# olydis/vlg_matching

Measured on AMD Instinct MI355X. Metric: vlg_queries_per_sec, higher is better.
Workload: dtype u32

## Files before the change

### vlg_matching_amd/csrc/join_device.hpp

```cpp
#pragma once
namespace {

constexpr uint32_t kNone = 0xFFFFFFFFu;
constexpr uint32_t kChecksumSlots = 64;

struct SegMeta {
    uint32_t begin, end;
    uint32_t pbegin, pend;
    uint32_t dist;
    uint32_t level;
    uint32_t next;
    uint32_t query;
    uint64_t lo, hi;
};

struct QueryMeta {
    uint32_t seg0;
    uint32_t k;
    uint64_t end_len;
    uint64_t out_first;
    uint64_t out_tuple;
};

__device__ __forceinline__ uint64_t sat_add(uint64_t a, uint64_t b) { uint64_t c = a + b; return c < a ? ~0ull : c; }
// ... 381 lines not shown
        }
        out[i] = v;
    }
}

template <typename pos_t>
__global__ void __launch_bounds__(256) join_init_kernel(const pos_t* __restrict__ P, const uint32_t* __restrict__ seg_begin, uint32_t nseg,
                                                        const SegMeta* __restrict__ sm, uint64_t r0, uint64_t r1, uint64_t* __restrict__ fbits,
                                                        pos_t* __restrict__ endp)
{
    const uint32_t lane = threadIdx.x & 63;
    const uint64_t wave = ((uint64_t)blockIdx.x * blockDim.x + threadIdx.x) >> 6;
    const uint64_t run_begin = r0 + wave * kRun;
    if (run_begin >= r1) return;
    const uint64_t run_end = run_begin + kRun < r1 ? run_begin + kRun : r1;
    uint32_t s_w = seg_find(seg_begin, nseg, run_begin);
    for (uint64_t base = run_begin; base < run_end; base += 64) {
        const uint64_t e = base + lane;
        if (e < run_end) {
            uint32_t s = s_w;
            while (seg_begin[s + 1] <= e) ++s;
            const SegMeta m = sm[s];
            endp[e] = P[phys_of(m, (uint32_t)e)];
            s_w = s;
        }
        const unsigned long long act = __ballot(e < run_end);
        if (lane == 0) fbits[base >> 6] = act;
        s_w = __shfl(s_w, 0);
    }
}

template <typename pos_t, bool kLast>
__device__ __forceinline__ bool link_finish(const pos_t* __restrict__ P, const SegMeta& nx, const FeasRef& fb, uint32_t e, bool want, uint32_t j,
                                            pos_t v, pos_t thi, pos_t* __restrict__ endp, uint32_t* __restrict__ link)
{
    bool ok = false;
    if (want && j < nx.pend) {
        if (kLast) {
            ok = v <= thi;
            if (ok) { if (link) link[e] = j; endp[e] = v; }
        } else {
            const uint32_t at = nx.begin + (j - nx.pbegin);
            const uint32_t ej = next_feasible(fb, at);
            if (ej < nx.end) {
                const pos_t pv = ej == at ? v : P[phys_of(nx, ej)];
                if (pv <= thi) { ok = true; if (link) link[e] = ej; endp[e] = endp[ej]; }
            }
        }
    }
    return ok;
}

template <typename pos_t, bool kLast>
__global__ void __launch_bounds__(256) join_link_kernel(const pos_t* __restrict__ P, const pos_t* __restrict__ F ,
                                                        const uint32_t* __restrict__ seg_begin, uint32_t nseg,
                                                        const SegMeta* __restrict__ sm, uint32_t r0, uint32_t r1,
                                                        FeasRef fb, uint64_t* __restrict__ fbits_out,
                                                        pos_t* __restrict__ endp, uint32_t* __restrict__ link)
{
    const uint32_t lane = threadIdx.x & 63;
    const uint64_t wave = ((uint64_t)blockIdx.x * blockDim.x + threadIdx.x) >> 6;
    if (wave * kLinkRun >= (uint64_t)(r1 - r0)) return;
    const uint32_t run_begin = r0 + (uint32_t)wave * kLinkRun;
    const uint32_t run_end = r1 - run_begin > kLinkRun ? run_begin + kLinkRun : r1;
    uint32_t s_w = wave_seg_find(seg_begin, nseg, run_begin);
    uint32_t seg_end = seg_begin[s_w + 1];
    SegMeta m = sm[s_w], nx = sm[m.next];
    uint32_t hint_seg = kNone, hint = 0;
    pos_t x_pre = 0, x_pre1 = 0;
    bool have_pre = false, have_pre1 = false;
    for (uint32_t base = run_begin; base < run_end; base += 64) {
        if (base >= seg_end) {
            while (seg_begin[s_w + 1] <= base) ++s_w;
            seg_end = seg_begin[s_w + 1];
            m = sm[s_w]; nx = sm[m.next];
            have_pre = false; have_pre1 = false;
        }
        if (run_end - base >= 128 && base + 127 < seg_end) {
            const uint32_t e0 = base + lane, e1 = e0 + 64;
            const pos_t x0 = have_pre ? x_pre : P[phys_of(m, e0)];
            const pos_t x1 = have_pre1 ? x_pre1 : P[phys_of(m, e1)];
            const uint32_t left = run_end - base - 128;
            const uint32_t room = seg_end - base - 128;
            have_pre = left > 0 && (left < 64 ? left : 64u) <= room;
            have_pre1 = left >= 128 && room >= 128;
            if (have_pre) x_pre = e0 + 128 < run_end ? P[phys_of(m, e0 + 128)] : (pos_t)0;
            if (have_pre1) x_pre1 = P[phys_of(m, e1 + 128)];
            pos_t tlo0, thi0, tlo1, thi1, v0 = 0, v1 = 0;
            const bool want0 = gap_window<pos_t>((uint64_t)x0, nx.lo, nx.hi, tlo0, thi0);
            const bool want1 = gap_window<pos_t>((uint64_t)x1, nx.lo, nx.hi, tlo1, thi1);
            uint32_t j0 = nx.pend, j1 = nx.pend;
            if (hint_seg != s_w)
                hint = wave_kary_lower_bound(P, F, nx.pbegin, nx.pend, (uint64_t)__shfl(tlo0, 0));
            wave_lower_bound2(P, F, hint, nx.pend, tlo0, want0, tlo1, want1, j0, v0, j1, v1);
            if (!want0) j0 = nx.pend;
            if (!want1) j1 = nx.pend;
            const bool ok0 = link_finish<pos_t, kLast>(P, nx, fb, e0, want0, j0, v0, thi0, endp, link);
            const bool ok1 = link_finish<pos_t, kLast>(P, nx, fb, e1, want1, j1, v1, thi1, endp, link);
            const unsigned long long okm0 = __ballot(ok0), okm1 = __ballot(ok1);
            if (lane == 0) { fbits_out[base >> 6] = okm0; fbits_out[(base >> 6) + 1] = okm1; }
            hint_seg = s_w;
            hint = __shfl(j1, 63);
            base += 64;
            continue;
        }
        have_pre1 = false;
        const uint32_t e = base + lane;
        const bool active = e < run_end;
        const uint32_t step_last = run_end - base > 64 ? base + 63 : run_end - 1;
        uint32_t j = 0, s_last = s_w;
        if (step_last < seg_end) {
            const pos_t x = have_pre ? x_pre : (active ? P[phys_of(m, e)] : (pos_t)0);
            const uint32_t en = e + 64;
            have_pre = run_end - base > 64 && (run_end - base > 128 ? base + 127 : run_end - 1) < seg_end;
            if (have_pre) x_pre = en < run_end ? P[phys_of(m, en)] : (pos_t)0;
            pos_t tlo, thi, v = 0;
            const bool want = gap_window<pos_t>((uint64_t)x, nx.lo, nx.hi, tlo, thi) && active;
            j = nx.pend;
            if (hint_seg != s_w) hint = wave_kary_lower_bound(P, F, nx.pbegin, nx.pend, (uint64_t)__shfl(tlo, 0));
            j = wave_lower_bound(P, F, hint, nx.pend, tlo, want, v);
            if (!want) j = nx.pend;
            const bool ok = link_finish<pos_t, kLast>(P, nx, fb, e, want, j, v, thi, endp, link);
            const unsigned long long okm = __ballot(ok);
            if (lane == 0) fbits_out[base >> 6] = okm;
        } else {
            have_pre = false;
            uint32_t s = s_w;
            bool ok = false;
            if (active) {
                while (seg_begin[s + 1] <= e) ++s;
                const SegMeta ml = sm[s];
                const SegMeta nl = sm[ml.next];
                const uint64_t x = P[phys_of(ml, e)];
                const uint64_t tlo = sat_add(x, nl.lo), thi = sat_add(x, nl.hi);
                j = gallop_lower_bound(P, (s == hint_seg) ? hint : nl.pbegin, nl.pend, tlo);
                if (e < ml.end) {
                    if (kLast) {
                        ok = j < nl.pend && (uint64_t)P[j] <= thi;
                        if (ok) { if (link) link[e] = j; endp[e] = P[j]; }
                    } else if (j < nl.pend) {
                        const uint32_t ej = next_feasible(fb, (uint64_t)nl.begin + (j - nl.pbegin));
                        if (ej < nl.end && (uint64_t)P[phys_of(nl, ej)] <= thi) { ok = true; if (link) link[e] = ej; endp[e] = endp[ej]; }
                    }
                }
            }
            const unsigned long long okm = __ballot(ok);
            if (lane == 0) fbits_out[base >> 6] = okm;
            s_last = __shfl(s, (int)(step_last - base));
        }
        hint_seg = s_last;
        hint = __shfl(j, (int)(step_last - base));
    }
}

template <typename pos_t>
__global__ void __launch_bounds__(256) join_jump_kernel(const pos_t* __restrict__ P, const pos_t* __restrict__ F, const uint32_t* __restrict__ seg_begin, uint32_t nseg,
                                                        const SegMeta* __restrict__ sm, const QueryMeta* __restrict__ qm, uint64_t r0,
                                                        uint64_t r1, FeasRef fb, const pos_t* __restrict__ endp,
                                                        uint32_t* __restrict__ jump, uint32_t* __restrict__ qstart)
{
    __shared__ pos_t s_tile[4][kTB];
    const uint32_t lane = threadIdx.x & 63, wv = threadIdx.x >> 6;
    const uint64_t wave = uniform(((uint64_t)blockIdx.x * blockDim.x + threadIdx.x) >> 6);
    const uint64_t run_begin = r0 + wave * kRun;
    if (run_begin >= r1) return;
    const uint64_t run_end = run_begin + kRun < r1 ? run_begin + kRun : r1;
    pos_t* tile = s_tile[wv];
    uint32_t s = wave_seg_find(seg_begin, nseg, run_begin);
    uint64_t cur = run_begin;
    while (cur < run_end) {
        while (seg_begin[s + 1] <= cur) ++s;
        const SegMeta m = sm[s];
        const uint64_t seg_end = seg_begin[s + 1];
        if (m.level != 0) {
            const uint64_t piece_end = run_end < seg_end ? run_end : seg_end;
            for (uint64_t a = cur + lane; a < piece_end; a += 64) jump[a] = kNone;
            cur = piece_end;
        } else if (m.end - m.begin >= kMinPiece && cur < m.end) {
            const uint64_t piece_end = run_end < m.end ? run_end : (uint64_t)m.end;
            const uint64_t end_len = qm[m.query].end_len;
            if (cur == m.begin && lane == 0) { const uint32_t me = next_feasible(fb, cur); qstart[m.query] = me < m.end ? me : kNone; }
            uint32_t fence = 0;
            for (uint64_t blk0 = cur; blk0 < piece_end; blk0 += kBlk) {
                const uint64_t blk1 = blk0 + kBlk < piece_end ? blk0 + kBlk : piece_end;
                pos_t key[kKeys], v[kKeys];
                uint32_t j[kKeys];
                uint32_t need = 0;
#pragma unroll
                for (uint32_t i = 0; i < kKeys; ++i) {
                    const uint64_t a = blk0 + lane + 64 * i;
                    key[i] = 0;
                    if (a < blk1 && is_feasible(fb, a)) {
                        pos_t unused;
                        if (gap_window<pos_t>((uint64_t)endp[a], end_len, end_len, key[i], unused)) need |= 1u << i;
                    }
                }
                const uint32_t own = phys_of(m, (uint32_t)blk0) + 1;
                fence = fence > own ? fence : own;
                const uint32_t asked = need;
                tile_lower_bounds<pos_t>(P, F, fence, m.pend, tile, key, need, j, v);
                uint32_t jm = fence;
#pragma unroll
                for (uint32_t i = 0; i < kKeys; ++i) {
                    const uint64_t a = blk0 + lane + 64 * i;
                    if (a < blk1) {
                        uint32_t out = kNone;
                        if ((asked >> i) & 1) {
                            jm = j[i] > jm ? j[i] : jm;
                            if (j[i] < m.pend) {
                                const uint32_t ej = next_feasible(fb, (uint64_t)m.begin + (j[i] - m.pbegin));
                                if (ej < m.end) out = ej;
                            }
                        }
                        jump[a] = out;
                    }
                }
                jm = wave_max_u32(jm);
                fence = jm;
            }
            cur = piece_end;
        } else {
            const uint64_t e = cur + lane;
            const uint64_t grp_end = cur + 64 < run_end ? cur + 64 : run_end;
            if (e < grp_end) {
                uint32_t sl = s;
                while (seg_begin[sl + 1] <= e) ++sl;
                const SegMeta ml = sm[sl];
                uint32_t out = kNone;
                if (ml.level == 0 && e < ml.end) {
                    if (is_feasible(fb, e)) {
                        const uint64_t lim = sat_add((uint64_t)endp[e], qm[ml.query].end_len);
                        const uint32_t jp = gallop_lower_bound(P, phys_of(ml, (uint32_t)e) + 1, ml.pend, lim);
                        if (jp < ml.pend) {
                            const uint32_t ej = next_feasible(fb, (uint64_t)ml.begin + (jp - ml.pbegin));
                            if (ej < ml.end) out = ej;
                        }
                    }
                    if ((uint32_t)e == ml.begin) { const uint32_t me = next_feasible(fb, e); qstart[ml.query] = me < ml.end ? me : kNone; }
                }
                jump[e] = out;
            }
            cur = grp_end;
        }
    }
}

constexpr uint32_t kTile = 1024;

__global__ void __launch_bounds__(256) chain_tiles_kernel(const uint32_t* __restrict__ jump, uint64_t t0 ,
                                                          uint64_t r1, uint2* __restrict__ xh)
{
    static_assert(kTile == 1024, "the packed word holds 10-bit tile offsets");
    __shared__ uint32_t s_ext[kTile];
    __shared__ uint32_t s_st[2][kTile];
    constexpr uint32_t kDone = 1u << 10;
    const uint64_t base = t0 + (uint64_t)blockIdx.x * kTile;
    const uint64_t tile_end = base + kTile;
    uint32_t st[4];
    bool open = false;
#pragma unroll
    for (uint32_t r = 0; r < 4; ++r) {
        const uint32_t li = threadIdx.x + 256 * r;
        const uint64_t e = base + li;
        const uint32_t j = e < r1 ? jump[e] : kNone;
        const bool inside = j != kNone && (uint64_t)j < tile_end;
        s_ext[li] = j;
        st[r] = (inside ? (uint32_t)(j - base) : kDone) | (li << 21);
        s_st[0][li] = st[r];
        open |= inside;
    }
    uint32_t cur = 0;
    for (uint32_t round = 0; round < 10 && __syncthreads_or(open); ++round) {
        open = false;
#pragma unroll
        for (uint32_t r = 0; r < 4; ++r) {
            const uint32_t li = threadIdx.x + 256 * r;
            if (!(st[r] & kDone)) {
                const uint32_t nx = s_st[cur][st[r] & 1023u];
                const uint32_t hops = ((st[r] >> 11) & 1023u) + ((nx >> 11) & 1023u) + 1;
                st[r] = (nx & 0x7FFu) | (hops << 11) | (nx & (1023u << 21));
                open |= !(st[r] & kDone);
            }
            s_st[cur ^ 1][li] = st[r];
        }
        cur ^= 1;
    }
    __syncthreads();
#pragma unroll
    for (uint32_t r = 0; r < 4; ++r) {
        const uint32_t li = threadIdx.x + 256 * r;
        const uint64_t e = base + li;
        if (e < r1) xh[e] = make_uint2(s_ext[st[r] >> 21], ((st[r] >> 11) & 1023u) + 1);
    }
}

__global__ void chain_walk_kernel(const SegMeta* __restrict__ sm, const QueryMeta* __restrict__ qm, uint32_t nq,
                                  const uint32_t* __restrict__ qstart, const uint2* __restrict__ xh, const uint32_t* __restrict__ rec_begin,
                                  uint2* __restrict__ records, uint32_t* __restrict__ rec_count, unsigned long long* __restrict__ counts)
{
    uint32_t q = blockIdx.x * blockDim.x + threadIdx.x;
    if (q >= nq) return;
    const QueryMeta Q = qm[q];
    unsigned long long n_match = 0;
    uint32_t nrec = 0;
    if (Q.seg0 != kNone) {
        const uint32_t mbegin = sm[Q.seg0].begin;
        uint2* rec = records + rec_begin[q];
        uint32_t cur = qstart[q];
        while (cur != kNone) {
            uint2 v = xh[cur];
            rec[nrec++] = make_uint2(cur, mbegin + (uint32_t)n_match);
            n_match += v.y;
            cur = v.x;
        }
    }
    rec_count[q] = nrec;
    counts[q] = n_match;
}

__global__ void __launch_bounds__(256) chain_emit_kernel(const uint32_t* __restrict__ rec_begin, const uint32_t* __restrict__ rec_count,
                                                         const uint2* __restrict__ records, uint32_t total_rec_slots,
                                                         const uint32_t* __restrict__ rec_query, const uint32_t* __restrict__ jump,
                                                         const uint2* __restrict__ xh, uint64_t r1 ,
                                                         uint32_t* __restrict__ mlist)
{
    constexpr uint16_t kOut = 0xFFFFu;
    constexpr uint32_t kPer = kTile / 64;
    __shared__ uint16_t s_t[4][2][kTile];
    const uint32_t lane = threadIdx.x & 63, wv = threadIdx.x >> 6;
    const uint32_t r = uniform((uint32_t)(((uint64_t)blockIdx.x * blockDim.x + threadIdx.x) >> 6));
    if (r >= total_rec_slots) return;
    const uint32_t q = rec_query[r];
    if (r - rec_begin[q] >= rec_count[q]) return;
    const uint2 rc = records[r];
    const uint64_t tile_base = (uint64_t)(rc.x / kTile) * kTile;
    const uint32_t cnt = uniform(xh[rc.x].y);
#pragma unroll
    for (uint32_t i = 0; i < kPer; ++i) {
        const uint64_t e = tile_base + lane + 64 * i;
        const uint32_t j = e < r1 ? jump[e] : kNone;
        s_t[wv][0][lane + 64 * i] = (j != kNone && (uint64_t)j < tile_base + kTile) ? (uint16_t)(j - (uint32_t)tile_base) : kOut;
// ... 94 lines not shown
```

### vlg_matching_amd/csrc/search.hip

```cpp
#include <algorithm>
#include <chrono>
#include <cstdio>
#include <cstdlib>
#include <cstring>
#include <mutex>
#include <numeric>
#include <thread>
#include <unordered_map>
#include <string.h>
#include <string>
#include <vector>
#include "common.hpp"
#include "kernels.hpp"
#include <rocprim/rocprim.hpp>

using namespace vlg;

#include "search_types.hpp"
#include "filter_shape.hpp"
#include "window_cut.hpp"
#include "shape_dispatch.hpp"

enum { KS_BSEARCH = 0, KS_EXPAND, KS_LOCATE, KS_LOCATE_PART, KS_LOCATE_RESOLVE, KS_SORT, KS_FILTER_LADDER, KS_FILTER_PIVOT, KS_FILTER_PASS, KS_FILTER_COMPACT,
       KS_JOIN_INIT, KS_JOIN_LINK, KS_JOIN_SCAN, KS_JOIN_CHAIN, KS_GATHER, KS_EXCHANGE, KS_WINDOW_CUT, KS_CLASS_SEARCH, KS_COUNT };
static const char* kKernelNames[KS_COUNT] = {"backward_search", "expand", "locate", "locate_partition", "locate_resolve", "sort", "filter_ladder", "filter_pivot",
                                             "filter_pass", "filter_compact", "join_init", "join_link", "join_scan", "join_chain", "gather", "exchange", "window_cut", "class_search"};

struct vlg_workspace {
    hipStream_t stream = nullptr;
    uint64_t cap_bytes = 0;
    uint8_t* arena = nullptr;
    uint64_t arena_bytes = 0;
    HostPool host;
    bool profile = false;
    bool dedup = true;
    bool sweep = true;
    bool tuples = true;
    bool trail = true;
    bool filter = true;
    uint64_t filter_min = 1ull << 12;
    uint64_t filter_stream_min = 1ull << 16;
    bool filter_pivot = true;
    uint64_t filter_group_bytes = 0;
    uint64_t filter_pivot_ratio = 3;
    uint64_t pivot_range_ratio = 16;
    uint32_t compact_dense_min = 256;
    uint32_t pivot_rungs = 1;
    int list_sort = 1;
    uint64_t global_sort_min = 1ull << 20;
    bool quad_walk = true;
    uint64_t sweep_min = 1ull << 22;
    uint64_t sweep_tail = 1ull << 22;
    uint32_t unsample_pct = 0;
    uint64_t unsample_min = 1ull << 28;
    uint64_t unsample_tail = 1ull << 20;
    uint32_t class_intervals = 1024;
    uint64_t sample_reads = 0;
    uint8_t* head = nullptr;
    uint64_t head_bytes = 0;
    uint64_t tmp_key[6] = {0, 0, 0, 0, 0, 0};
    size_t tmp_bytes = 0;
    int x_ranks = 1, x_rank = 0;
    vlg_exchange_fn x_fn = nullptr;
    vlg_alltoall_fn x_a2a = nullptr;
    void* x_ctx = nullptr;
    void* x_comm = nullptr;
    bool exchange_all = false;
    uint64_t* x_status = nullptr;
    uint32_t x_agreed = 0;
    vlg_kernel_stat stats[KS_COUNT];
    std::vector<std::pair<hipEvent_t, hipEvent_t>> pending[KS_COUNT];
    std::vector<hipEvent_t> free_events;
};

namespace {

struct PhaseTrace {
    bool on, sync;
    hipStream_t st;
    std::chrono::steady_clock::time_point t0;
    explicit PhaseTrace(hipStream_t s) : on(getenv("VLG_TRACE") != nullptr), sync(!on || strcmp(getenv("VLG_TRACE"), "host") != 0), st(s), t0(std::chrono::steady_clock::now()) {}
    void mark(const char* what)
    {
// ... 110 lines not shown
}

extern "C" void vlg_workspace_destroy(vlg_workspace* ws)
{
    if (!ws) return;
    ws_collect(ws);
    for (hipEvent_t e : ws->free_events) (void)hipEventDestroy(e);
    if (ws->arena) (void)hipFree(ws->arena);
    if (ws->head) (void)hipFree(ws->head);
    if (ws->x_status) (void)hipFree(ws->x_status);
    ws->host.release();
    delete ws;
}

extern "C" vlg_status vlg_workspace_profile(vlg_workspace* ws, int enable)
{
    if (!ws) return fail(VLG_E_INVALID, "null argument");
    ws_reset_stats(ws);
    ws->profile = enable != 0;
    return VLG_OK;
}

extern "C" vlg_status vlg_workspace_set_option(vlg_workspace* ws, const char* name, int64_t value)
{
    if (!ws || !name) return fail(VLG_E_INVALID, "null argument");
    if (!strcmp(name, "dedup")) { ws->dedup = value != 0; return VLG_OK; }
    if (!strcmp(name, "sweep")) { ws->sweep = value != 0; return VLG_OK; }
    if (!strcmp(name, "sweep_min")) { ws->sweep_min = (uint64_t)value; return VLG_OK; }
    if (!strcmp(name, "global_sort_min")) { ws->global_sort_min = (uint64_t)value; return VLG_OK; }
    if (!strcmp(name, "list_sort")) { ws->list_sort = value > 2 ? 1 : (int)value; return VLG_OK; }
    if (!strcmp(name, "trail")) { ws->trail = value != 0; return VLG_OK; }
    if (!strcmp(name, "quad_walk")) { ws->quad_walk = value != 0; return VLG_OK; }
    if (!strcmp(name, "tuples")) { ws->tuples = value != 0; return VLG_OK; }
    if (!strcmp(name, "filter")) { ws->filter = value != 0; return VLG_OK; }
    if (!strcmp(name, "filter_min")) { ws->filter_min = (uint64_t)value; return VLG_OK; }
    if (!strcmp(name, "filter_pivot")) { ws->filter_pivot = value != 0; return VLG_OK; }
    if (!strcmp(name, "filter_pivot_ratio")) { ws->filter_pivot_ratio = (uint64_t)value; return VLG_OK; }
    if (!strcmp(name, "pivot_range_ratio")) { ws->pivot_range_ratio = (uint64_t)std::max<int64_t>(0, value); return VLG_OK; }
    if (!strcmp(name, "compact_dense_min")) { ws->compact_dense_min = (uint32_t)std::max<int64_t>(0, std::min<int64_t>(value, 1 << 20)); return VLG_OK; }
    if (!strcmp(name, "pivot_rungs")) { ws->pivot_rungs = value <= 0 ? 0u : (value == 1 ? 1u : 2u); return VLG_OK; }
    if (!strcmp(name, "filter_stream_min")) { ws->filter_stream_min = (uint64_t)value; return VLG_OK; }
    if (!strcmp(name, "filter_group_bytes")) { ws->filter_group_bytes = (uint64_t)value; return VLG_OK; }
    if (!strcmp(name, "reserve")) {
        const uint64_t b = std::min<uint64_t>((uint64_t)value, ws->cap_bytes);
        return ws_reserve(ws, b + b / 96 + (256ull << 20));
    }
    if (!strcmp(name, "sweep_tail")) { ws->sweep_tail = (uint64_t)value; return VLG_OK; }
    if (!strcmp(name, "exchange_all")) { ws->exchange_all = value != 0; return VLG_OK; }
    if (!strcmp(name, "unsample_pct")) { ws->unsample_pct = (uint32_t)std::max<int64_t>(0, std::min<int64_t>(value, 1 << 20)); return VLG_OK; }
    if (!strcmp(name, "unsample_tail")) { ws->unsample_tail = (uint64_t)value; return VLG_OK; }
    if (!strcmp(name, "class_intervals")) {
        if (value < 1 || value > (int64_t)kClassIntervalsMax) return fail(VLG_E_INVALID, "class_intervals: 1 .. 2^20");
        ws->class_intervals = (uint32_t)value;
        return VLG_OK;
    }
    if (!strcmp(name, "unsample_min")) { ws->unsample_min = (uint64_t)value; return VLG_OK; }
    return fail(VLG_E_INVALID, std::string("unknown workspace option ") + name);
}

namespace {
vlg_status ws_exchange_reset(vlg_workspace* ws, int n_ranks)
{
    ws->x_comm = nullptr; ws->x_fn = nullptr; ws->x_a2a = nullptr; ws->x_ctx = nullptr; ws->x_ranks = 1; ws->x_rank = 0;
    if (n_ranks > 1 && !ws->x_status) VLG_HIP_TRY(hipMalloc((void**)&ws->x_status, 8 * 1024));
    return VLG_OK;
}
// ... 871 lines not shown
            hipLaunchKernelGGL(HIP_KERNEL_NAME(fence_build_kernel<pos_t>), launch_grid(gacc / 64, 8192), dim3(256), 0, st, L.P, (uint64_t)0, gacc / 64, L.F);
            VLG_HIP_TRY(hipGetLastError());
        }
        return VLG_OK;
    }
};

template <typename pos_t>
vlg_status build_physical(const vlg_index* idx, vlg_workspace* ws, vlg_result* res, const Plan& pl, const SuperChunk& sc, const ChunkPlan& cp, bool wide,
                          Arena& A, unsigned long long* d_stats, Lists<pos_t>& L, const vlg_queries* q = nullptr, const std::vector<uint64_t>* xq = nullptr,
                          Agreement* ag = nullptr)
{
    L.P = L.Pc = L.F = L.R = nullptr; L.pc_cap = 0; L.roff = nullptr;
    PhysicalPass<pos_t> pp{idx, ws, res, pl, cp, wide, A, d_stats, L};
    pp.layout(sc.dlist);
    if (!pp.gacc) return ag ? ag->settle(VLG_OK) : VLG_OK;
    const std::function<vlg_status()> plan_sort = [&pp]() { return pp.plan_sort(); };
    if (vlg_status s = pp.carve()) return s;
    if (vlg_status s = pp.locate(plan_sort)) return s;
    if (vlg_status s = pp.sort(L.P)) return s;
    if (vlg_status s = pp.exchange(L.P, q, xq, ag)) return s;
    if (vlg_status s = pp.check_sort()) return s;
    if (vlg_status s = pp.fences_and_ladder()) return s;
    res->sum.located_occurrences += pp.acc;
    return VLG_OK;
}

}

#include "filter.hpp"

namespace {

template <typename pos_t>
struct JoinChunk {
    const vlg_queries* q; vlg_workspace* ws; vlg_result* res; const uint64_t q0, q1; const Plan& pl; const Lists<pos_t>& L;
    Arena A;
    unsigned long long* d_stats; const FilterGroup* fg;
    hipStream_t st = ws->stream;
    PhaseTrace jt{st};
    const pos_t* P = L.P;
    pos_t* Pc = L.Pc;
    const pos_t* F = L.F;
    const uint64_t s0 = q->qsub[q0], s1 = q->qsub[q1];
    const uint32_t nseg = (uint32_t)(s1 - s0), nq = (uint32_t)(q1 - q0);
    ResultPiece piece{q0, q1};
    bool empty = false;
    svec<QueryMeta> qm;
    uint32_t kmax = 0, nlive = 0, n_rec = 0;
    svec<uint32_t> t_seg, t_cidx; svec<uint64_t> t_run0;
    bool t_kind[2] = {false, false};
    uint64_t pc_total = 0;
    std::vector<uint32_t> cls_count, cls_first;
    std::vector<uint64_t> cls_slot_begin, cls_slot_end;
    svec<SegMeta> sm; svec<uint32_t> seg_begin;
    uint64_t T = 0, lvl0_begin = 0, lvl0_end = 0, t0 = 0;
    svec<uint32_t> rec_begin, rec_query;
    svec<unsigned long long> counts, first_of;
    uint32_t* link = nullptr; pos_t* endp = nullptr;
    FeasBits fb; uint64_t* lvl_ptr[kBitLevels]; FeasBits* d_fb = nullptr; FeasRef fref{nullptr, nullptr};
    uint32_t* jump = nullptr; uint32_t* mlist = nullptr; uint2* xh = nullptr;
    SegMeta* d_sm = nullptr; QueryMeta* d_qm = nullptr; uint32_t* d_segb = nullptr; unsigned long long* d_counts = nullptr;
    uint32_t* d_qstart = nullptr; uint32_t* d_recb = nullptr; uint32_t* d_recc = nullptr; uint32_t* d_recq = nullptr; uint2* d_rec = nullptr;

    uint64_t eo(uint64_t s) const { return fg ? fg->eff[s - fg->sub0] : pl.occ[s]; }
    bool filtered(uint64_t s) const { return fg && fg->cidx[s - fg->sub0] != kNone; }
    bool live(uint64_t qi) const { return q->qsub[qi + 1] > q->qsub[qi] && eo(q->qsub[qi]) > 0; }

    void survivor_tasks()
    {
        qm.resize(nq);
        if (fg) { t_seg.reserve(nseg); t_cidx.reserve(nseg); t_run0.reserve(nseg + 1); }
        t_run0.push_back(0);
        for (uint64_t qi = q0; qi < q1; ++qi) {
            const uint64_t a = q->qsub[qi];
            const uint32_t k = (uint32_t)(q->qsub[qi + 1] - a);
            QueryMeta& Q = qm[qi - q0];
            Q.k = k; Q.end_len = q->end_len[qi]; Q.out_first = Q.out_tuple = 0; Q.seg0 = kNone;
            if (!live(qi)) continue;
            kmax = std::max(kmax, k);
            if (fg && !fg->speculated)
                for (uint32_t i = 0; i < k; ++i) {
                    const uint32_t c = fg->cidx[a + i - fg->sub0];
                    if (c == kNone) continue;
                    t_cidx.push_back(c);
                    t_seg.push_back(fg->cseg[c]);
                    t_kind[fg->ckind[c]] = true;
                    t_run0.push_back(t_run0.back() + (fg->crun0[c + 1] - fg->crun0[c]));
                    pc_total += fg->eff[a + i - fg->sub0];
                }
        }
    }

    vlg_status compact_survivors()
    {
        if (t_seg.empty()) return VLG_OK;
// ... 81 lines not shown
                cnt = (m0.end - 1) / kTile - m0.begin / kTile + 1;
            }
            rec_begin[i + 1] = rec_begin[i] + cnt;
            rec_query.insert(rec_query.end(), cnt, i);
        }
        n_rec = rec_begin[nq];
        empty = lvl0_end <= lvl0_begin;
        t0 = lvl0_begin / kTile * kTile;
    }

    vlg_status carve()
    {
        link = ws->tuples ? A.take<uint32_t>(T) : nullptr;
        endp = A.take<pos_t>(T);
        uint64_t words = (T + 63) / 64 + 1;
        for (uint32_t l = 0; l < kBitLevels; ++l) {
            fb.lvl[l] = lvl_ptr[l] = A.take<uint64_t>(words);
            fb.words[l] = words;
            words = (words + 63) / 64 + 1;
        }
        d_fb = A.take<FeasBits>(1);
        fref = FeasRef{lvl_ptr[0], d_fb};
        const uint64_t n0 = lvl0_end - t0;
        uint32_t* jump_a = A.take<uint32_t>(n0);
        uint32_t* mlist_a = A.take<uint32_t>(n0);
        uint2* xh_a = A.take<uint2>(n0);
        jump = jump_a ? jump_a - t0 : nullptr;
        mlist = mlist_a ? mlist_a - t0 : nullptr;
        xh = xh_a ? xh_a - t0 : nullptr;
        d_sm = A.take<SegMeta>(nlive + 1);
        d_qm = A.take<QueryMeta>(nq);
        d_segb = A.take<uint32_t>(nlive + 2);
        d_counts = A.take<unsigned long long>(nq);
        d_qstart = A.take<uint32_t>(nq);
        d_recb = A.take<uint32_t>(nq + 1);
        d_recc = A.take<uint32_t>(nq);
        d_recq = A.take<uint32_t>(n_rec + 1);
        d_rec = A.take<uint2>(n_rec + 1);
        if (A.failed) return fail(VLG_E_INTERNAL, "arena carve failed (join)");
        return VLG_OK;
    }

    vlg_status upload()
    {
        for (uint32_t l = 0; l < kBitLevels; ++l) VLG_HIP_TRY(hipMemsetAsync(lvl_ptr[l], 0, fb.words[l] * 8, st));
        VLG_HIP_TRY(hipMemcpyAsync(d_fb, &fb, sizeof fb, hipMemcpyHostToDevice, st));
        VLG_HIP_TRY(hipMemcpyAsync(d_recb, rec_begin.data(), (nq + 1) * 4, hipMemcpyHostToDevice, st));
        if (n_rec) VLG_HIP_TRY(hipMemcpyAsync(d_recq, rec_query.data(), n_rec * 4, hipMemcpyHostToDevice, st));
        VLG_HIP_TRY(hipMemsetAsync(d_qstart, 0xFF, nq * 4, st));
        VLG_HIP_TRY(hipMemcpyAsync(d_sm, sm.data(), (nlive + 1) * sizeof(SegMeta), hipMemcpyHostToDevice, st));
        VLG_HIP_TRY(hipMemcpyAsync(d_segb, seg_begin.data(), (nlive + 2) * 4, hipMemcpyHostToDevice, st));
        VLG_HIP_TRY(hipMemcpyAsync(d_qm, qm.data(), nq * sizeof(QueryMeta), hipMemcpyHostToDevice, st));
        return VLG_OK;
    }

    vlg_status summarize_class(uint32_t d)
    {
        const uint64_t b0 = cls_slot_begin[d], b1 = cls_slot_end[d];
        if (b1 <= b0) return VLG_OK;
        Timed t(ws, KS_JOIN_SCAN, (b1 - b0) / 8);
        uint64_t w0 = b0 >> 6, w1 = (b1 + 63) >> 6;
        for (uint32_t l = 1; l < kBitLevels; ++l) {
            w0 >>= 6; w1 = (w1 + 63) >> 6;
            hipLaunchKernelGGL(bits_summary_kernel, launch_grid(w1 - w0, 4096), dim3(256), 0, st, fb.lvl[l - 1], fb.words[l - 1], w0, w1, lvl_ptr[l]);
        }
        VLG_HIP_TRY(hipGetLastError());
        return VLG_OK;
    }

    vlg_status link_classes()
    {
        if (cls_slot_end[0] > cls_slot_begin[0]) {
            Timed t(ws, KS_JOIN_INIT, 0);
            hipLaunchKernelGGL(HIP_KERNEL_NAME(join_init_kernel<pos_t>), dim3(runs_grid(cls_slot_end[0] - cls_slot_begin[0])), dim3(256), 0, st, P,
                               d_segb, nlive, d_sm, cls_slot_begin[0], cls_slot_end[0], lvl_ptr[0], endp);
        }
        if (vlg_status s = summarize_class(0)) return s;
        for (uint32_t dist = 1; dist < kmax; ++dist) {
            const uint64_t b0 = cls_slot_begin[dist], b1 = cls_slot_end[dist];
            if (b1 > b0) {
                Timed t(ws, KS_JOIN_LINK, 8ull * (b1 - b0));
                const auto kernel = dist == 1 ? join_link_kernel<pos_t, true> : join_link_kernel<pos_t, false>;
                hipLaunchKernelGGL(kernel, dim3(runs_grid(b1 - b0, kLinkRun)), dim3(256), 0, st, P, F, d_segb, nlive, d_sm, (uint32_t)b0, (uint32_t)b1, fref,
                                   lvl_ptr[0], endp, link);
            }
            if (vlg_status s = summarize_class(dist)) return s;
        }
        return VLG_OK;
    }

    vlg_status chain()
    {
        {
            Timed t(ws, KS_JOIN_CHAIN, 8ull * (lvl0_end - lvl0_begin));
            hipLaunchKernelGGL(HIP_KERNEL_NAME(join_jump_kernel<pos_t>), dim3(runs_grid(lvl0_end - lvl0_begin)), dim3(256), 0, st, P, F, d_segb, nlive, d_sm,
                               d_qm, lvl0_begin, lvl0_end, fref, endp, jump, d_qstart);
            if (t0 < lvl0_begin) VLG_HIP_TRY(hipMemsetAsync(jump + t0, 0xFF, (lvl0_begin - t0) * 4, st));
            hipLaunchKernelGGL(chain_tiles_kernel, dim3((uint32_t)((lvl0_end - t0 + kTile - 1) / kTile)), dim3(256), 0, st, jump, t0, lvl0_end, xh);
            hipLaunchKernelGGL(chain_walk_kernel, dim3((nq + 63) / 64), dim3(64), 0, st, d_sm, d_qm, nq, d_qstart, xh, d_recb, d_rec, d_recc,
                               d_counts);
            if (n_rec)
                hipLaunchKernelGGL(chain_emit_kernel, dim3((n_rec + 3) / 4), dim3(256), 0, st, d_recb, d_recc, d_rec, n_rec, d_recq, jump, xh, lvl0_end, mlist);
        }
        VLG_HIP_TRY(hipGetLastError());
        return VLG_OK;
    }

    vlg_status gather()
    {
        counts.resize(nq);
        VLG_HIP_TRY(hipMemcpyAsync(counts.data(), d_counts, nq * 8, hipMemcpyDeviceToHost, st));
        VLG_HIP_TRY(hipStreamSynchronize(st));
        jt.mark("  chunk: link + chain");
        uint64_t M = 0, TV = 0;
        for (uint32_t i = 0; i < nq; ++i) {
            qm[i].out_first = M; qm[i].out_tuple = TV;
            M += counts[i]; TV += ws->tuples ? counts[i] * qm[i].k : 0;
            res->counts[q0 + i] = counts[i];
        }
        piece.matches = M; piece.tuple_vals = TV;
        if (M) {
            piece.width = sizeof(pos_t);
            VLG_HIP_TRY(result_alloc(&piece.d_first, M * sizeof(pos_t), &piece.first_bytes));
            if (TV) VLG_HIP_TRY(result_alloc(&piece.d_tuples, TV * sizeof(pos_t), &piece.tuple_bytes));
            res->pieces.push_back(piece);
            jt.mark("  chunk: result malloc");
            VLG_HIP_TRY(hipMemcpyAsync(d_qm, qm.data(), nq * sizeof(QueryMeta), hipMemcpyHostToDevice, st));
            first_of.resize(nq);
            for (uint32_t i = 0; i < nq; ++i) first_of[i] = qm[i].out_first;
            VLG_HIP_TRY(hipMemcpyAsync(d_counts, first_of.data(), nq * 8, hipMemcpyHostToDevice, st));
            Timed t(ws, KS_GATHER, sizeof(pos_t) * (M + TV));
            hipLaunchKernelGGL(HIP_KERNEL_NAME(join_gather_kernel<pos_t>), dim3(runs_grid(M)), dim3(256), 0, st, P, d_sm, d_qm, d_counts, nq, M, link, mlist,
                               static_cast<pos_t*>(piece.d_first), static_cast<pos_t*>(piece.d_tuples), d_stats + kStatsChecksum);
// ... 1174 lines not shown
```

### vlg_matching_amd/variants.py

```python
import os
import subprocess
from concurrent.futures import ThreadPoolExecutor

_HERE = os.path.dirname(os.path.abspath(__file__))
ROOT = os.path.dirname(_HERE)
CSRC = os.path.join(_HERE, "csrc")

DEFAULTS = {
    "VLG_LINK_RUN": 2048, "VLG_COOP_WINDOWS2": 4, "VLG_RUNG_SHIFT": 2, "VLG_RESOLVE_HOPS": 4096, "VLG_RESOLVE_CHUNK": 4096,
    "VLG_GROUP_CHUNK": 2048, "VLG_STAGE_LISTS": 1, "VLG_SWEEP_PAIRS": 1, "VLG_PIVOT_GROUPS": 2, "VLG_PIVOT_TURNS": 1,
    "VLG_COMPACT_RUNS": 16, "VLG_SPARSE_TURN": 8, "VLG_SORT_CLASSES": 5, "VLG_BUCKET_SORT": 1, "VLG_WINDOW_SORT": 1,
    "VLG_WINDOWS_PER_TILE": 2, "VLG_WINDOW_RANK_LOOP": 0, "VLG_WINDOW_THREADS": 256, "VLG_WINDOW_ITEMS": 12, "VLG_FETCH_THREADS": 16,
}

VARIANTS = {
    "small": {"VLG_LINK_RUN": 192, "VLG_RESOLVE_CHUNK": 256, "VLG_GROUP_CHUNK": 256, "VLG_RESOLVE_HOPS": 2, "VLG_COMPACT_RUNS": 1,
              "VLG_SPARSE_TURN": 1, "VLG_PIVOT_GROUPS": 1, "VLG_COOP_WINDOWS2": 1},
    "alternates": {"VLG_SORT_CLASSES": 3, "VLG_SWEEP_PAIRS": 0, "VLG_STAGE_LISTS": 0, "VLG_WINDOW_RANK_LOOP": 1, "VLG_WINDOWS_PER_TILE": 4,
                   "VLG_PIVOT_TURNS": 4, "VLG_RUNG_SHIFT": 4},
    "radix": {"VLG_BUCKET_SORT": 0, "VLG_RUNG_SHIFT": 3},
}

ENV_RUNS = {
    "env_paths": {"VLG_RESOLVE_GROUPED": "0", "VLG_SWEEP_LOOKAHEAD": "0", "VLG_NO_SPECULATIVE_COMPACT": "1", "VLG_WINDOW_SORT": "0"},
}


def constants(name):
    c = dict(DEFAULTS)
    if name is not None:
        c.update(VARIANTS[name])
    return c


def extra_defs(name):
    return " ".join("-D%s=%d" % kv for kv in sorted(VARIANTS[name].items()))


def library(name):
    return os.path.join(ROOT, "build", "variants", name, "libvlg_hip.so")


def build(name, jobs=4):
    subprocess.check_call(["make", "-C", CSRC, "-j%d" % jobs, "variant", "VARIANT=" + name, "EXTRA_DEFS=" + extra_defs(name)],
                          stdout=subprocess.DEVNULL)


def build_all(jobs=None):
    jobs = jobs or max(1, min(8, (os.cpu_count() or 4) // len(VARIANTS)))
    with ThreadPoolExecutor(len(VARIANTS)) as ex:
        for f in [ex.submit(build, n, jobs) for n in VARIANTS]:
            f.result()
```

Baseline: 773,600.

## Fuse level-0 jump target computation into the join link kernel

The link kernel now computes jump targets for level-0 segments directly, using a shared-memory stretch of upcoming positions plus a far lower-bound fallback. This replaces most of the separate jump-kernel pass and avoids re-reading endp for level-0 elements. Feasibility adjustment of jump targets moves into chain_tiles, and qstart is computed inside chain_walk instead of being stored in a buffer. The cost is extra shared memory, more register pressure and more branching in the link kernel, plus extra memsets for gaps between distance classes.

```diff
diff --git a/vlg_matching_amd/csrc/join_device.hpp b/vlg_matching_amd/csrc/join_device.hpp
--- a/vlg_matching_amd/csrc/join_device.hpp
+++ b/vlg_matching_amd/csrc/join_device.hpp
@@ -437,40 +437,90 @@
 
 template <typename pos_t, bool kLast>
 __device__ __forceinline__ bool link_finish(const pos_t* __restrict__ P, const SegMeta& nx, const FeasRef& fb, uint32_t e, bool want, uint32_t j,
-                                            pos_t v, pos_t thi, pos_t* __restrict__ endp, uint32_t* __restrict__ link)
+                                            pos_t v, pos_t thi, pos_t* __restrict__ endp, uint32_t* __restrict__ link, bool store_end, pos_t& end)
 {
     bool ok = false;
     if (want && j < nx.pend) {
         if (kLast) {
             ok = v <= thi;
-            if (ok) { if (link) link[e] = j; endp[e] = v; }
+            if (ok) { if (link) link[e] = j; if (store_end) endp[e] = v; end = v; }
         } else {
             const uint32_t at = nx.begin + (j - nx.pbegin);
             const uint32_t ej = next_feasible(fb, at);
             if (ej < nx.end) {
                 const pos_t pv = ej == at ? v : P[phys_of(nx, ej)];
-                if (pv <= thi) { ok = true; if (link) link[e] = ej; endp[e] = endp[ej]; }
+                if (pv <= thi) { ok = true; if (link) link[e] = ej; end = endp[ej]; if (store_end) endp[e] = end; }
             }
         }
     }
     return ok;
 }
 
-template <typename pos_t, bool kLast>
+constexpr uint32_t kStretch = 256;
+
+template <typename pos_t>
+__device__ __noinline__ uint32_t jump_far_lower_bound(const pos_t* __restrict__ P, const pos_t* __restrict__ F, uint32_t wb, uint32_t b, pos_t key, bool need)
+{
+    uint32_t j = b;
+    pos_t v = 0;
+    wave_far_lower_bound(P, F, wb < b ? wb : b, b, key, need, j, v);
+    return j < b ? j : b;
+}
+
+template <typename pos_t, uint32_t kN>
+__device__ __forceinline__ void stretch_jump_targets(const pos_t* __restrict__ P, const pos_t* __restrict__ F, const SegMeta& m, uint32_t pb,
+                                                     const pos_t* __restrict__ tile, const pos_t (&key)[kN], const bool (&need)[kN], uint32_t (&out)[kN])
+{
+    const uint32_t lane = threadIdx.x & 63;
+    const pos_t tile_last = tile[kStretch - 1];
+    uint32_t pos[kN];
+    bool far[kN], any_far = false;
+#pragma unroll
+    for (uint32_t i = 0; i < kN; ++i) { pos[i] = 0; far[i] = need[i] && key[i] > tile_last; any_far |= far[i]; }
+#pragma unroll
+    for (uint32_t step = kStretch / 2; step; step >>= 1) {
+#pragma unroll
+        for (uint32_t i = 0; i < kN; ++i)
+            if (tile[pos[i] + step - 1] < key[i]) pos[i] += step;
+    }
+    uint32_t j[kN];
+#pragma unroll
+    for (uint32_t i = 0; i < kN; ++i) {
+        const uint32_t own = 64 * i + lane;
+        j[i] = pb + (pos[i] > own ? pos[i] : own + 1);
+    }
+    if (__any(any_far)) {
+#pragma unroll
+        for (uint32_t i = 0; i < kN; ++i) {
+            const uint32_t jf = jump_far_lower_bound<pos_t>(P, F, pb + kStretch, m.pend, key[i], far[i]);
+            if (far[i]) j[i] = jf;
+        }
+    }
+#pragma unroll
+    for (uint32_t i = 0; i < kN; ++i) out[i] = need[i] && j[i] < m.pend ? m.begin + (j[i] - m.pbegin) : kNone;
+}
+
+template <typename pos_t, bool kLast, bool kJump>
 __global__ void __launch_bounds__(256) join_link_kernel(const pos_t* __restrict__ P, const pos_t* __restrict__ F ,
                                                         const uint32_t* __restrict__ seg_begin, uint32_t nseg,
                                                         const SegMeta* __restrict__ sm, uint32_t r0, uint32_t r1,
                                                         FeasRef fb, uint64_t* __restrict__ fbits_out,
-                                                        pos_t* __restrict__ endp, uint32_t* __restrict__ link)
-{
+                                                        pos_t* __restrict__ endp, uint32_t* __restrict__ link,
+                                                        const QueryMeta* __restrict__ qm, uint32_t jlo, uint32_t jhi, uint32_t* __restrict__ jump)
+{
+    __shared__ pos_t s_stretch[kJump ? 4 : 1][kJump ? kStretch : 1];
+    constexpr pos_t kInf = (pos_t)~(pos_t)0;
     const uint32_t lane = threadIdx.x & 63;
     const uint64_t wave = ((uint64_t)blockIdx.x * blockDim.x + threadIdx.x) >> 6;
     if (wave * kLinkRun >= (uint64_t)(r1 - r0)) return;
+    pos_t* const tile = s_stretch[kJump ? threadIdx.x >> 6 : 0];
     const uint32_t run_begin = r0 + (uint32_t)wave * kLinkRun;
     const uint32_t run_end = r1 - run_begin > kLinkRun ? run_begin + kLinkRun : r1;
     uint32_t s_w = wave_seg_find(seg_begin, nseg, run_begin);
     uint32_t seg_end = seg_begin[s_w + 1];
     SegMeta m = sm[s_w], nx = sm[m.next];
+    bool lvl0 = kJump && m.level == 0;
+    uint64_t end_len = lvl0 ? qm[m.query].end_len : 0;
     uint32_t hint_seg = kNone, hint = 0;
     pos_t x_pre = 0, x_pre1 = 0;
     bool have_pre = false, have_pre1 = false;
@@ -479,6 +529,8 @@
             while (seg_begin[s_w + 1] <= base) ++s_w;
             seg_end = seg_begin[s_w + 1];
             m = sm[s_w]; nx = sm[m.next];
+            lvl0 = kJump && m.level == 0;
+            end_len = lvl0 ? qm[m.query].end_len : 0;
             have_pre = false; have_pre1 = false;
         }
         if (run_end - base >= 128 && base + 127 < seg_end) {
@@ -489,8 +541,13 @@
             const uint32_t room = seg_end - base - 128;
             have_pre = left > 0 && (left < 64 ? left : 64u) <= room;
             have_pre1 = left >= 128 && room >= 128;
-            if (have_pre) x_pre = e0 + 128 < run_end ? P[phys_of(m, e0 + 128)] : (pos_t)0;
-            if (have_pre1) x_pre1 = P[phys_of(m, e1 + 128)];
+            if (lvl0) {
+                x_pre = e0 + 128 < m.end ? P[phys_of(m, e0 + 128)] : kInf;
+                x_pre1 = e1 + 128 < m.end ? P[phys_of(m, e1 + 128)] : kInf;
+            } else {
+                if (have_pre) x_pre = e0 + 128 < run_end ? P[phys_of(m, e0 + 128)] : (pos_t)0;
+                if (have_pre1) x_pre1 = P[phys_of(m, e1 + 128)];
+            }
             pos_t tlo0, thi0, tlo1, thi1, v0 = 0, v1 = 0;
             const bool want0 = gap_window<pos_t>((uint64_t)x0, nx.lo, nx.hi, tlo0, thi0);
             const bool want1 = gap_window<pos_t>((uint64_t)x1, nx.lo, nx.hi, tlo1, thi1);
@@ -500,10 +557,27 @@
             wave_lower_bound2(P, F, hint, nx.pend, tlo0, want0, tlo1, want1, j0, v0, j1, v1);
             if (!want0) j0 = nx.pend;
             if (!want1) j1 = nx.pend;
-            const bool ok0 = link_finish<pos_t, kLast>(P, nx, fb, e0, want0, j0, v0, thi0, endp, link);
-            const bool ok1 = link_finish<pos_t, kLast>(P, nx, fb, e1, want1, j1, v1, thi1, endp, link);
+            pos_t end0 = 0, end1 = 0;
+            const bool ok0 = link_finish<pos_t, kLast>(P, nx, fb, e0, want0, j0, v0, thi0, endp, link, !lvl0, end0);
+            const bool ok1 = link_finish<pos_t, kLast>(P, nx, fb, e1, want1, j1, v1, thi1, endp, link, !lvl0, end1);
             const unsigned long long okm0 = __ballot(ok0), okm1 = __ballot(ok1);
             if (lane == 0) { fbits_out[base >> 6] = okm0; fbits_out[(base >> 6) + 1] = okm1; }
+            if (kJump) {
+                if (lvl0) {
+                    pos_t key[2] = {0, 0}, unused;
+                    const bool need[2] = {ok0 && gap_window<pos_t>((uint64_t)end0, end_len, end_len, key[0], unused),
+                                          ok1 && gap_window<pos_t>((uint64_t)end1, end_len, end_len, key[1], unused)};
+                    tile[lane] = x0; tile[64 + lane] = x1; tile[128 + lane] = x_pre; tile[192 + lane] = x_pre1;
+                    wave_sync();
+                    uint32_t out[2];
+                    stretch_jump_targets<pos_t, 2>(P, F, m, phys_of(m, base), tile, key, need, out);
+                    wave_sync();
+                    jump[e0] = out[0]; jump[e1] = out[1];
+                } else {
+                    if (e0 >= jlo && e0 < jhi) jump[e0] = kNone;
+                    if (e1 >= jlo && e1 < jhi) jump[e1] = kNone;
+                }
+            }
             hint_seg = s_w;
             hint = __shfl(j1, 63);
             base += 64;
@@ -525,9 +599,26 @@
             if (hint_seg != s_w) hint = wave_kary_lower_bound(P, F, nx.pbegin, nx.pend, (uint64_t)__shfl(tlo, 0));
             j = wave_lower_bound(P, F, hint, nx.pend, tlo, want, v);
             if (!want) j = nx.pend;
-            const bool ok = link_finish<pos_t, kLast>(P, nx, fb, e, want, j, v, thi, endp, link);
+            pos_t end = 0;
+            const bool ok = link_finish<pos_t, kLast>(P, nx, fb, e, want, j, v, thi, endp, link, !lvl0, end);
             const unsigned long long okm = __ballot(ok);
             if (lane == 0) fbits_out[base >> 6] = okm;
+            if (kJump) {
+                if (lvl0) {
+                    pos_t key[1] = {0}, unused;
+                    const bool need[1] = {ok && gap_window<pos_t>((uint64_t)end, end_len, end_len, key[0], unused)};
+                    tile[lane] = active ? x : (e < m.end ? P[phys_of(m, e)] : kInf);
+#pragma unroll
+                    for (uint32_t r = 1; r < kStretch / 64; ++r) tile[64 * r + lane] = e + 64 * r < m.end ? P[phys_of(m, e + 64 * r)] : kInf;
+                    wave_sync();
+                    uint32_t out[1];
+                    stretch_jump_targets<pos_t, 1>(P, F, m, phys_of(m, base), tile, key, need, out);
+                    wave_sync();
+                    if (active) jump[e] = out[0];
+                } else if (active && e >= jlo && e < jhi) {
+                    jump[e] = kNone;
+                }
+            }
         } else {
             have_pre = false;
             uint32_t s = s_w;
@@ -539,14 +630,29 @@
                 const uint64_t x = P[phys_of(ml, e)];
                 const uint64_t tlo = sat_add(x, nl.lo), thi = sat_add(x, nl.hi);
                 j = gallop_lower_bound(P, (s == hint_seg) ? hint : nl.pbegin, nl.pend, tlo);
+                const bool first = kJump && ml.level == 0;
+                pos_t end = 0;
                 if (e < ml.end) {
                     if (kLast) {
                         ok = j < nl.pend && (uint64_t)P[j] <= thi;
-                        if (ok) { if (link) link[e] = j; endp[e] = P[j]; }
+                        if (ok) { if (link) link[e] = j; end = P[j]; if (!first) endp[e] = end; }
                     } else if (j < nl.pend) {
                         const uint32_t ej = next_feasible(fb, (uint64_t)nl.begin + (j - nl.pbegin));
-                        if (ej < nl.end && (uint64_t)P[phys_of(nl, ej)] <= thi) { ok = true; if (link) link[e] = ej; endp[e] = endp[ej]; }
+                        if (ej < nl.end && (uint64_t)P[phys_of(nl, ej)] <= thi) {
+                            ok = true;
+                            if (link) link[e] = ej;
+                            end = endp[ej];
+                            if (!first) endp[e] = end;
+                        }
                     }
+                }
+                if (kJump && e >= jlo && e < jhi) {
+                    uint32_t out = kNone;
+                    if (first && ok) {
+                        const uint32_t jp = gallop_lower_bound(P, phys_of(ml, e) + 1, ml.pend, sat_add((uint64_t)end, qm[ml.query].end_len));
+                        if (jp < ml.pend) out = ml.begin + (jp - ml.pbegin);
+                    }
+                    jump[e] = out;
                 }
             }
             const unsigned long long okm = __ballot(ok);
@@ -562,7 +668,7 @@
 __global__ void __launch_bounds__(256) join_jump_kernel(const pos_t* __restrict__ P, const pos_t* __restrict__ F, const uint32_t* __restrict__ seg_begin, uint32_t nseg,
                                                         const SegMeta* __restrict__ sm, const QueryMeta* __restrict__ qm, uint64_t r0,
                                                         uint64_t r1, FeasRef fb, const pos_t* __restrict__ endp,
-                                                        uint32_t* __restrict__ jump, uint32_t* __restrict__ qstart)
+                                                        uint32_t* __restrict__ jump)
 {
     __shared__ pos_t s_tile[4][kTB];
     const uint32_t lane = threadIdx.x & 63, wv = threadIdx.x >> 6;
@@ -584,7 +690,6 @@
         } else if (m.end - m.begin >= kMinPiece && cur < m.end) {
             const uint64_t piece_end = run_end < m.end ? run_end : (uint64_t)m.end;
             const uint64_t end_len = qm[m.query].end_len;
-            if (cur == m.begin && lane == 0) { const uint32_t me = next_feasible(fb, cur); qstart[m.query] = me < m.end ? me : kNone; }
             uint32_t fence = 0;
             for (uint64_t blk0 = cur; blk0 < piece_end; blk0 += kBlk) {
                 const uint64_t blk1 = blk0 + kBlk < piece_end ? blk0 + kBlk : piece_end;
@@ -641,7 +746,6 @@
                             if (ej < ml.end) out = ej;
                         }
                     }
-                    if ((uint32_t)e == ml.begin) { const uint32_t me = next_feasible(fb, e); qstart[ml.query] = me < ml.end ? me : kNone; }
                 }
                 jump[e] = out;
             }
@@ -651,23 +755,64 @@
 }
 
 constexpr uint32_t kTile = 1024;
-
-__global__ void __launch_bounds__(256) chain_tiles_kernel(const uint32_t* __restrict__ jump, uint64_t t0 ,
-                                                          uint64_t r1, uint2* __restrict__ xh)
+constexpr uint32_t kTileFeasWords = 32;
+
+__global__ void __launch_bounds__(256) chain_tiles_kernel(uint32_t* __restrict__ jump, uint64_t t0 ,
+                                                          uint64_t r1, FeasRef fb, const uint32_t* __restrict__ seg_begin, uint32_t nseg,
+                                                          uint2* __restrict__ xh)
 {
     static_assert(kTile == 1024, "the packed word holds 10-bit tile offsets");
     __shared__ uint32_t s_ext[kTile];
     __shared__ uint32_t s_st[2][kTile];
     constexpr uint32_t kDone = 1u << 10;
+    __shared__ uint64_t s_fb[kTileFeasWords];
     const uint64_t base = t0 + (uint64_t)blockIdx.x * kTile;
     const uint64_t tile_end = base + kTile;
+    uint32_t jw[4];
+#pragma unroll
+    for (uint32_t r = 0; r < 4; ++r) {
+        const uint64_t e = base + threadIdx.x + 256 * r;
+        jw[r] = e < r1 ? jump[e] : kNone;
+    }
+    const uint64_t w_base = base >> 6;
+    if (threadIdx.x < kTileFeasWords) s_fb[threadIdx.x] = w_base + threadIdx.x <= ((r1 - 1) >> 6) ? fb.lvl0[w_base + threadIdx.x] : 0;
+    __syncthreads();
+    uint32_t moved = 0;
+#pragma unroll
+    for (uint32_t r = 0; r < 4; ++r) {
+        const uint32_t j = jw[r];
+        if (j != kNone) {
+            const uint64_t wi = ((uint64_t)j >> 6) - w_base;
+            const uint64_t bits = wi < kTileFeasWords ? s_fb[wi] >> (j & 63) : 0;
+            const uint32_t ej = bits ? j + (uint32_t)__ffsll((long long)bits) - 1 : next_feasible(fb, j);
+            moved |= (uint32_t)(ej != j) << r;
+            jw[r] = ej;
+        }
+    }
+    if (__any(moved != 0)) {
+        const uint32_t s_t = wave_seg_find(seg_begin, nseg, base);
+        const uint32_t t_next = seg_begin[s_t + 1];
+#pragma unroll
+        for (uint32_t r = 0; r < 4; ++r) {
+            const uint64_t e = base + threadIdx.x + 256 * r;
+            if ((moved >> r) & 1) {
+                uint32_t lim = t_next;
+                if ((uint64_t)lim < tile_end) {
+                    uint32_t s = s_t;
+                    while (seg_begin[s + 1] <= e) ++s;
+                    lim = seg_begin[s + 1];
+                }
+                if (jw[r] >= lim) jw[r] = kNone;
+                jump[e] = jw[r];
+            }
+        }
+    }
     uint32_t st[4];
     bool open = false;
 #pragma unroll
     for (uint32_t r = 0; r < 4; ++r) {
         const uint32_t li = threadIdx.x + 256 * r;
-        const uint64_t e = base + li;
-        const uint32_t j = e < r1 ? jump[e] : kNone;
+        const uint32_t j = jw[r];
         const bool inside = j != kNone && (uint64_t)j < tile_end;
         s_ext[li] = j;
         st[r] = (inside ? (uint32_t)(j - base) : kDone) | (li << 21);
@@ -699,8 +844,8 @@
     }
 }
 
-__global__ void chain_walk_kernel(const SegMeta* __restrict__ sm, const QueryMeta* __restrict__ qm, uint32_t nq,
-                                  const uint32_t* __restrict__ qstart, const uint2* __restrict__ xh, const uint32_t* __restrict__ rec_begin,
+__global__ void chain_walk_kernel(const SegMeta* __restrict__ sm, const QueryMeta* __restrict__ qm, uint32_t nq, FeasRef fb,
+                                  const uint2* __restrict__ xh, const uint32_t* __restrict__ rec_begin,
                                   uint2* __restrict__ records, uint32_t* __restrict__ rec_count, unsigned long long* __restrict__ counts)
 {
     uint32_t q = blockIdx.x * blockDim.x + threadIdx.x;
@@ -709,9 +854,10 @@
     unsigned long long n_match = 0;
     uint32_t nrec = 0;
     if (Q.seg0 != kNone) {
-        const uint32_t mbegin = sm[Q.seg0].begin;
+        const uint32_t mbegin = sm[Q.seg0].begin, mend = sm[Q.seg0].end;
         uint2* rec = records + rec_begin[q];
-        uint32_t cur = qstart[q];
+        uint32_t cur = mbegin < mend ? next_feasible(fb, mbegin) : kNone;
+        if (cur >= mend) cur = kNone;
         while (cur != kNone) {
             uint2 v = xh[cur];
             rec[nrec++] = make_uint2(cur, mbegin + (uint32_t)n_match);
diff --git a/vlg_matching_amd/csrc/search.hip b/vlg_matching_amd/csrc/search.hip
--- a/vlg_matching_amd/csrc/search.hip
+++ b/vlg_matching_amd/csrc/search.hip
@@ -49,6 +49,7 @@
     int list_sort = 1;
     uint64_t global_sort_min = 1ull << 20;
     bool quad_walk = true;
+    bool fuse_jump = true;
     uint64_t sweep_min = 1ull << 22;
     uint64_t sweep_tail = 1ull << 22;
     uint32_t unsample_pct = 0;
@@ -225,6 +226,7 @@
     if (!strcmp(name, "trail")) { ws->trail = value != 0; return VLG_OK; }
     if (!strcmp(name, "quad_walk")) { ws->quad_walk = value != 0; return VLG_OK; }
     if (!strcmp(name, "tuples")) { ws->tuples = value != 0; return VLG_OK; }
+    if (!strcmp(name, "fuse_jump")) { ws->fuse_jump = value != 0; return VLG_OK; }
     if (!strcmp(name, "filter")) { ws->filter = value != 0; return VLG_OK; }
     if (!strcmp(name, "filter_min")) { ws->filter_min = (uint64_t)value; return VLG_OK; }
     if (!strcmp(name, "filter_pivot")) { ws->filter_pivot = value != 0; return VLG_OK; }
@@ -1162,6 +1164,8 @@
 
 namespace {
 
+inline bool fuse_jump_env() { static const bool on = [] { const char* e = getenv("VLG_FUSE_JUMP"); return !(e && e[0] == '0'); }(); return on; }
+
 template <typename pos_t>
 struct JoinChunk {
     const vlg_queries* q; vlg_workspace* ws; vlg_result* res; const uint64_t q0, q1; const Plan& pl; const Lists<pos_t>& L;
@@ -1176,6 +1180,7 @@
     const uint32_t nseg = (uint32_t)(s1 - s0), nq = (uint32_t)(q1 - q0);
     ResultPiece piece{q0, q1};
     bool empty = false;
+    const bool fused = ws->fuse_jump && fuse_jump_env();
     svec<QueryMeta> qm;
     uint32_t kmax = 0, nlive = 0, n_rec = 0;
     svec<uint32_t> t_seg, t_cidx; svec<uint64_t> t_run0;
@@ -1191,7 +1196,7 @@
     FeasBits fb; uint64_t* lvl_ptr[kBitLevels]; FeasBits* d_fb = nullptr; FeasRef fref{nullptr, nullptr};
     uint32_t* jump = nullptr; uint32_t* mlist = nullptr; uint2* xh = nullptr;
     SegMeta* d_sm = nullptr; QueryMeta* d_qm = nullptr; uint32_t* d_segb = nullptr; unsigned long long* d_counts = nullptr;
-    uint32_t* d_qstart = nullptr; uint32_t* d_recb = nullptr; uint32_t* d_recc = nullptr; uint32_t* d_recq = nullptr; uint2* d_rec = nullptr;
+    uint32_t* d_recb = nullptr; uint32_t* d_recc = nullptr; uint32_t* d_recq = nullptr; uint2* d_rec = nullptr;
 
     uint64_t eo(uint64_t s) const { return fg ? fg->eff[s - fg->sub0] : pl.occ[s]; }
     bool filtered(uint64_t s) const { return fg && fg->cidx[s - fg->sub0] != kNone; }
@@ -1339,7 +1344,6 @@
         d_qm = A.take<QueryMeta>(nq);
         d_segb = A.take<uint32_t>(nlive + 2);
         d_counts = A.take<unsigned long long>(nq);
-        d_qstart = A.take<uint32_t>(nq);
         d_recb = A.take<uint32_t>(nq + 1);
         d_recc = A.take<uint32_t>(nq);
         d_recq = A.take<uint32_t>(n_rec + 1);
@@ -1354,7 +1358,6 @@
         VLG_HIP_TRY(hipMemcpyAsync(d_fb, &fb, sizeof fb, hipMemcpyHostToDevice, st));
         VLG_HIP_TRY(hipMemcpyAsync(d_recb, rec_begin.data(), (nq + 1) * 4, hipMemcpyHostToDevice, st));
         if (n_rec) VLG_HIP_TRY(hipMemcpyAsync(d_recq, rec_query.data(), n_rec * 4, hipMemcpyHostToDevice, st));
-        VLG_HIP_TRY(hipMemsetAsync(d_qstart, 0xFF, nq * 4, st));
         VLG_HIP_TRY(hipMemcpyAsync(d_sm, sm.data(), (nlive + 1) * sizeof(SegMeta), hipMemcpyHostToDevice, st));
         VLG_HIP_TRY(hipMemcpyAsync(d_segb, seg_begin.data(), (nlive + 2) * 4, hipMemcpyHostToDevice, st));
         VLG_HIP_TRY(hipMemcpyAsync(d_qm, qm.data(), nq * sizeof(QueryMeta), hipMemcpyHostToDevice, st));
@@ -1386,10 +1389,12 @@
         for (uint32_t dist = 1; dist < kmax; ++dist) {
             const uint64_t b0 = cls_slot_begin[dist], b1 = cls_slot_end[dist];
             if (b1 > b0) {
+                const bool jumps = fused && b0 < lvl0_end && b1 > lvl0_begin;
                 Timed t(ws, KS_JOIN_LINK, 8ull * (b1 - b0));
-                const auto kernel = dist == 1 ? join_link_kernel<pos_t, true> : join_link_kernel<pos_t, false>;
+                const auto kernel = jumps ? (dist == 1 ? join_link_kernel<pos_t, true, true> : join_link_kernel<pos_t, false, true>)
+                                          : (dist == 1 ? join_link_kernel<pos_t, true, false> : join_link_kernel<pos_t, false, false>);
                 hipLaunchKernelGGL(kernel, dim3(runs_grid(b1 - b0, kLinkRun)), dim3(256), 0, st, P, F, d_segb, nlive, d_sm, (uint32_t)b0, (uint32_t)b1, fref,
-                                   lvl_ptr[0], endp, link);
+                                   lvl_ptr[0], endp, link, d_qm, (uint32_t)lvl0_begin, (uint32_t)lvl0_end, jump);
             }
             if (vlg_status s = summarize_class(dist)) return s;
         }
@@ -1400,12 +1405,19 @@
     {
         {
             Timed t(ws, KS_JOIN_CHAIN, 8ull * (lvl0_end - lvl0_begin));
-            hipLaunchKernelGGL(HIP_KERNEL_NAME(join_jump_kernel<pos_t>), dim3(runs_grid(lvl0_end - lvl0_begin)), dim3(256), 0, st, P, F, d_segb, nlive, d_sm,
-                               d_qm, lvl0_begin, lvl0_end, fref, endp, jump, d_qstart);
+            const uint64_t jb = fused ? std::max(cls_slot_begin[0], lvl0_begin) : lvl0_begin, je = fused ? cls_slot_end[0] : lvl0_end;
+            if (je > jb)
+                hipLaunchKernelGGL(HIP_KERNEL_NAME(join_jump_kernel<pos_t>), dim3(runs_grid(je - jb)), dim3(256), 0, st, P, F, d_segb, nlive, d_sm, d_qm, jb,
+                                   je, fref, endp, jump);
             if (t0 < lvl0_begin) VLG_HIP_TRY(hipMemsetAsync(jump + t0, 0xFF, (lvl0_begin - t0) * 4, st));
-            hipLaunchKernelGGL(chain_tiles_kernel, dim3((uint32_t)((lvl0_end - t0 + kTile - 1) / kTile)), dim3(256), 0, st, jump, t0, lvl0_end, xh);
-            hipLaunchKernelGGL(chain_walk_kernel, dim3((nq + 63) / 64), dim3(64), 0, st, d_sm, d_qm, nq, d_qstart, xh, d_recb, d_rec, d_recc,
-                               d_counts);
+            if (fused)
+                for (uint32_t d = 1; d < kmax; ++d) {
+                    const uint64_t p0 = std::max(cls_slot_end[d], lvl0_begin), p1 = std::min(cls_slot_begin[d - 1], lvl0_end);
+                    if (p1 > p0) VLG_HIP_TRY(hipMemsetAsync(jump + p0, 0xFF, (p1 - p0) * 4, st));
+                }
+            hipLaunchKernelGGL(chain_tiles_kernel, dim3((uint32_t)((lvl0_end - t0 + kTile - 1) / kTile)), dim3(256), 0, st, jump, t0, lvl0_end, fref, d_segb,
+                               nlive, xh);
+            hipLaunchKernelGGL(chain_walk_kernel, dim3((nq + 63) / 64), dim3(64), 0, st, d_sm, d_qm, nq, fref, xh, d_recb, d_rec, d_recc, d_counts);
             if (n_rec)
                 hipLaunchKernelGGL(chain_emit_kernel, dim3((n_rec + 3) / 4), dim3(256), 0, st, d_recb, d_recc, d_rec, n_rec, d_recq, jump, xh, lvl0_end, mlist);
         }
diff --git a/vlg_matching_amd/variants.py b/vlg_matching_amd/variants.py
--- a/vlg_matching_amd/variants.py
+++ b/vlg_matching_amd/variants.py
@@ -22,7 +22,8 @@
 }
 
 ENV_RUNS = {
-    "env_paths": {"VLG_RESOLVE_GROUPED": "0", "VLG_SWEEP_LOOKAHEAD": "0", "VLG_NO_SPECULATIVE_COMPACT": "1", "VLG_WINDOW_SORT": "0"},
+    "env_paths": {"VLG_RESOLVE_GROUPED": "0", "VLG_SWEEP_LOOKAHEAD": "0", "VLG_NO_SPECULATIVE_COMPACT": "1", "VLG_WINDOW_SORT": "0",
+                  "VLG_FUSE_JUMP": "0"},
 }
 
 
```

After: 815,700 (median of 6 runs). 5.4% higher.
